# mako443/Text2Pos-CVPR2022

Hardware: AMD Instinct MI355X
Metric: cells+queries encoded/sec and top-k retrieval QPS, 256-pt cells, 12k-cell DB (higher is better)
Workload: dtype f16x3 (fp32 operands split hi+lo into fp16, 3 f16 MFMAs, fp32 accumulate; fp32-class error) for the encoders / f64 MFMA for the ranking

## Files before the change

include/t2p.h:

```cpp
#ifndef T2P_H
#define T2P_H
#include <stddef.h>
#include <stdint.h>

#ifdef __cplusplus
extern "C" {
#endif

#define T2P_ABI_VERSION 31
#define T2P_DEFAULT_CHUNK_OBJECTS 65000
#define T2P_MAX_CHUNK_OBJECTS 65535
#define T2P_TUNING_MASK 0x5
#define T2P_E_ARG (-1)
#define T2P_E_WORKSPACE (-2)
#define T2P_E_UNSUPPORTED (-3)

typedef void* t2p_stream_t;

int t2p_abi_version(void);
const char* t2p_last_error(void);

typedef struct t2p_cell_weights {
    const float* sa_w1[3];
    const float* sa_b1[3];
    const float* sa_w2[3];
    const float* sa_b2[3];
    const float* ga_w1;
    const float* ga_b1;
    const float* ga_w2;
    const float* ga_b2;
    const float* lin1_w;
    const float* lin1_b;
    const float* lin2_w;
    const float* lin2_b;
    const float* pn_w;
    const float* pn_b;
    const float* col_w1;
    const float* col_b1;
    const float* col_w2;
    const float* col_b2;
    const float* pos_w1;
    const float* pos_b1;
    const float* pos_w2;
    const float* pos_b2;
    const float* merge_w;
    const float* merge_b;
    const float* g_wp;
    const float* g_bp;
    const float* g_wq;
    const float* g_w2;
    const float* g_b2;
    const float* lin_w1;
    const float* lin_b1;
    const float* lin_w2;
    const float* lin_b2;
    const void* sa_w2_x3[3];
    const void* ga_w2_x3;
    const float* sa_b2_x3[3];
    float sa_w2_scale[3];
    const void* lin1_x3;
    const void* lin2_x3;
    const void* merge_x3;
    const void* pn_x3;
    const void* g_wp_x3;
    const void* g_wq_x3;
// ... 204 lines not shown
```

text2pos-cvpr2022_amd/csrc/api.hip:

```cpp
#include <stdarg.h>
#include <stdlib.h>
#include <string.h>

#include <mutex>
#include <set>
#include <utility>

#include "../../include/t2p.h"
#include "t2p_common.h"

namespace t2p {

static thread_local char g_err[512] = "";

void set_error(const char* fmt, ...) {
    va_list ap;
    va_start(ap, fmt);
    vsnprintf(g_err, sizeof(g_err), fmt, ap);
    va_end(ap);
}

int num_cus() {
    static int cached = 0;
    if (cached == 0) {
// ... 294 lines not shown
            p.k_live = Geo::C[l - 1] + 4;
            p.W = W.sa_w1[l];
            p.W_x3 = cfg.precision == 1 ? W.sa_w1_x3[l] : nullptr;
            p.ldw = H;
            p.bias = W.sa_b1[l];
            p.out = ws.A[l];
            p.ldo = H;
            p.relu = 0;
            p.M = n * g.nd[l];
            p.amax_out = gslot(l == 1 ? G_A2 : G_A3);
            T2P_TRY(launch_ws(WS_DENSE_STORE, Geo::LD[l - 1] - (cfg.precision == 1 ? 16 : 0), H, p, st));
        }
        SaParams p{};
        p.A = ws.A[l];
        p.Bc = ws.B[l];
        p.wp = lds_btab[l] ? W.sa_w1[l] + (size_t)cf * Geo::H[l] : nullptr;
        p.W = W.sa_w2[l];
        p.W_x3 = cfg.precision == 1 ? W.sa_w2_x3[l] : nullptr;
        p.bias = cfg.precision == 1 ? W.sa_b2_x3[l] : W.sa_b2[l];
        p.out_scale = cfg.precision == 1 ? 1.0f / W.sa_w2_scale[l] : 1.0f;
        p.out = ws.F[l];
        p.ldo = Geo::LD[l];
        p.rows = ws.gt.rows[l];
        p.n_rows = ws.gt.n_rows[l];
        p.first = ws.first;
        p.fps_idx = ws.gt.fps_idx[l];
        p.pos_src = pos_src;
        p.ld_pos = ld_pos;
        p.pos_col0 = pos_col0;
        if (l == 0 && sa1_points) {
            p.feat_src = rgb;
            p.w1 = W.sa_w1[0];
            p.b1 = W.sa_b1[0];
        }
        p.n_dense = g.nd[l];
        p.n_cent = g.nc[l];
        p.n_obj = n;
        p.prefix_ws = ws.prefix[l];
        p.bounds_ws = ws.bounds[l];
        p.balanced = 1;
        p.amax_out = gslot(G_F1 + l);
        if (l == 2) p.out_rows = g.gp;
        T2P_TRY(launch_ws_sa(H, C, p, st));
    }
    {
        WsParams p{};
        p.A = ws.F[2];
        p.lda = Geo::LD[2];
        p.W = W.ga_w1;
        p.W_x3 = cfg.precision == 1 ? W.ga_w1_x3 : nullptr;
        p.ldw = 512;
        p.bias = W.ga_b1;
        p.out = ws.gh;
        _Float16* gh_hi = (_Float16*)ws.gh;
        _Float16* gh_lo = gh_hi + (size_t)gh_rows(n, g) * 512;
        if (cfg.precision == 1) {
            p.out_hi = gh_hi;
            p.out_lo = gh_lo;
            p.amax_out = gslot(G_GA_H);
        }
        p.ldo = 512;
        p.relu = 1;
        p.M = n * g.gp;
        T2P_TRY(launch_ws(WS_DENSE_STORE, Geo::LD[2] - (cfg.precision == 1 ? 16 : 0), 512, p, st));
        WsParams q{};
        q.A = ws.gh;
        if (cfg.precision == 1) {
            q.A_hi = gh_hi;
            q.A_lo = gh_lo;
        }
        q.lda = 512;
        q.W = W.ga_w2;
        q.W_x3 = cfg.precision == 1 ? W.ga_w2_x3 : nullptr;
        q.ldw = 1024;
        q.bias = W.ga_b2;
        q.out = ws.f0;
        q.ldo = 1024;
        q.relu = 1;
        q.M = n * g.gp;
        q.group_rows = g.gp;
        T2P_TRY(launch_ws(WS_DENSE_GROUPMAX, 512, 1024, q, st));
    }
    if (cfg.precision == 1 && W.lin1_x3 && W.lin2_x3) {
        T2P_TRY(launch_gemm_x3(ws.f0, 1024, W.lin1_x3, W.lin1_scale, W.lin1_b, ws.f1, 512, 0, n, 1024, 512, 1, st, nullptr, 0, gslot(G_PN_F0)));
        T2P_TRY(launch_gemm_x3(ws.f1, 512, W.lin2_x3, W.lin2_scale, W.lin2_b, ws.f2, 256, 0, n, 512, 256, 1, st, nullptr, 0, gslot(G_PN_F1)));
    } else {
        T2P_TRY(launch_gemm(ws.f0, 1024, W.lin1_w, W.lin1_b, ws.f1, 512, 0, n, 1024, 512, 1, st));
        T2P_TRY(launch_gemm(ws.f1, 512, W.lin2_w, W.lin2_b, ws.f2, 256, 0, n, 512, 256, 1, st));
    }
    }
    if (trunk_only) {
        T2P_TRY(copy_trace(tr->features0, ws.f0, (size_t)n * 1024, st));
        T2P_TRY(copy_trace(tr->features1, ws.f1, (size_t)n * 512, st));
        T2P_TRY(copy_trace(tr->features2, ws.f2, (size_t)n * 256, st));
        T2P_TRY(launch_guard_check(guard, cfg.overflow_flag, gbounds, st));
        return 0;
    }
    const int nfeat = (cfg.use_class ? 1 : 0) + (cfg.use_color ? 1 : 0) + (cfg.use_position ? 1 : 0);
    const int ldcat = nfeat * D;
    int slot = 0;
    if (cfg.use_class && cfg.class_embed) {
        T2P_TRY(launch_gather_rownorm(W.class_embedding, cfg.class_idx + o_lo, n, D, ws.cat, ldcat, slot * D, st));
        slot++;
    } else if (cfg.use_class) {
        const float* fin = cfg.pointnet_features == 0 ? ws.f0 : (cfg.pointnet_features == 1 ? ws.f1 : ws.f2);
        const int kin = cfg.pointnet_features == 0 ? 1024 : (cfg.pointnet_features == 1 ? 512 : 256);
        if (cfg.precision == 1 && W.pn_x3)
            T2P_TRY(launch_gemm_x3(fin, kin, W.pn_x3, W.pn_scale, W.pn_b, ws.P, D, 0, n, kin, D, 1, st, nullptr, 0,
                                          gslot(G_PN_F0 + cfg.pointnet_features)));
        else
            T2P_TRY(launch_gemm(fin, kin, W.pn_w, W.pn_b, ws.P, D, 0, n, kin, D, 1, st));
        T2P_TRY(launch_rownorm(ws.P, D, n, D, ws.cat, ldcat, slot * D, st));
        slot++;
    }
    if (cfg.use_color && cfg.color_embed) {
        T2P_TRY(launch_gather_rownorm(W.color_embedding, cfg.color_idx + o_lo, n, D, ws.cat, ldcat, slot * D, st));
        slot++;
    } else if (cfg.use_color) {
        T2P_TRY(launch_mlp3_norm(mean_rgb, n, W.col_w1, W.col_b1, W.col_w2, W.col_b2, D, ws.cat, ldcat, slot * D, st));
        slot++;
    }
    if (cfg.use_position) {
// ... 665 lines not shown
```

text2pos-cvpr2022_amd/csrc/ga2.hip:

```cpp
#include "t2p_common.h"

namespace t2p {
namespace {


constexpr int K = 512, NW = 128, NT = 512;
constexpr int KH = K / 2;
constexpr int S16_FULL = K / 16;
constexpr int LDHH = K + 8;
constexpr int PLANE = 32 * LDHH;
constexpr int TILE_HALVES = 2 * PLANE;
constexpr int XCH_FLOATS = 4 * 16 * 64;
constexpr size_t kLds = (size_t)2 * TILE_HALVES * 2 + (size_t)XCH_FLOATS * 4;
constexpr int CHUNKS = (2 * 32 * (K / 8)) / NT;

template <int GP>
__global__ __launch_bounds__(NT, 2) void k_ga2(WsParams p, int n_slices) {
    extern __shared__ __attribute__((aligned(16))) float lds[];
    _Float16* tile = (_Float16*)lds;
    float* xch = (float*)(tile + 2 * TILE_HALVES);

    const int tid = threadIdx.x, lane = tid & 63, wave = tid >> 6;
    const int wn = wave & 3, kh = wave >> 2;

    const int lin = blockIdx.x, nblk = gridDim.x;
    int slice, stream, n_streams;
    if ((nblk % (8 * n_slices)) == 0) {
        const int xcd = lin & 7, j = lin >> 3, per_xcd = nblk >> 3;
        slice = j % n_slices;
        stream = xcd * (per_xcd / n_slices) + j / n_slices;
        n_streams = nblk / n_slices;
    } else {
        slice = lin % n_slices;
        stream = lin / n_slices;
        n_streams = nblk / n_slices;
    }
    const int ncol0 = slice * NW + wn * 32;

    constexpr int S32 = KH / 32;
    const int q16 = lane >> 4, i16 = lane & 15;
    half8 w_hi[2][S32], w_lo[2][S32];
    {
        const uint4* wp = (const uint4*)p.W_x3;
        const int plane_u4 = (p.ldw / 32) * S16_FULL * 64;
#pragma unroll
        for (int cb = 0; cb < 2; cb++)
#pragma unroll
            for (int s = 0; s < S32; s++) {
                const int idx = (((ncol0 / 32) * S16_FULL + (8 * q16 + s)) * 2 + kh) * 32 + 16 * cb + i16;
                w_hi[cb][s] = __builtin_bit_cast(half8, wp[idx]);
                w_lo[cb][s] = __builtin_bit_cast(half8, wp[plane_u4 + idx]);
            }
    }
    float bias2[2];
#pragma unroll
    for (int cb = 0; cb < 2; cb++) bias2[cb] = p.bias ? p.bias[ncol0 + 16 * cb + i16] : 0.f;

    typedef __attribute__((address_space(3))) void lds_void;
    typedef const __attribute__((address_space(1))) void gl_void;
    auto dma_piece = [&](int64_t g, int buf, int it) {
        const int q = it * (NT / 64) + wave;
        const int pl = q >> 5, row = q & 31;
        const _Float16* base = (const _Float16*)(pl ? p.A_lo : p.A_hi);
        const _Float16* src = base + (g * 32 + row) * (int64_t)p.lda + lane * 8;
        _Float16* dst = tile + buf * TILE_HALVES + pl * PLANE + row * LDHH;
        __builtin_amdgcn_global_load_lds((gl_void*)src, (lds_void*)dst, 16, 0, 0);
    };
    auto dma_tile = [&](int64_t g, int buf) {
#pragma unroll
        for (int it = 0; it < CHUNKS; it++) dma_piece(g, buf, it);
    };
    int64_t g = stream;
    if (g < p.n_groups) dma_tile(g, 0);
    __syncthreads();
    for (int i = 0; g < p.n_groups; g += n_streams, i++) {
        const int64_t gn = g + n_streams;
        const bool more = gn < p.n_groups;

        typedef float f32x4v __attribute__((ext_vector_type(4)));
        const f32x4v kZero4 = {0.f, 0.f, 0.f, 0.f};
        f32x4v acc[4], accx[4];
        const _Float16* hrow = tile + (i & 1) * TILE_HALVES + i16 * LDHH + kh * KH + q16 * 64;
        half8 a_hi[2], a_lo[2];
#pragma unroll
        for (int rb = 0; rb < 2; rb++) {
            a_hi[rb] = *(const half8*)(hrow + rb * 16 * LDHH);
            a_lo[rb] = *(const half8*)(hrow + PLANE + rb * 16 * LDHH);
        }
#pragma unroll
        for (int sl = 0; sl < 4 * S32; sl++) {
            const int s = sl >> 2, b = sl & 3, rb = b >> 1, cb = b & 1;
            __builtin_amdgcn_sched_barrier(0);
            if (s + 1 < S32 && b == 2) {
                a_hi[0] = *(const half8*)(hrow + (s + 1) * 8);
                a_lo[0] = *(const half8*)(hrow + PLANE + (s + 1) * 8);
            }
            if (s > 0 && b == 0) {
                a_hi[1] = *(const half8*)(hrow + 16 * LDHH + s * 8);
                a_lo[1] = *(const half8*)(hrow + PLANE + 16 * LDHH + s * 8);
            }
            acc[b] = __builtin_amdgcn_mfma_f32_16x16x32_f16(a_hi[rb], w_hi[cb][s], s == 0 ? kZero4 : acc[b], 0, 0, 0);
            accx[b] = __builtin_amdgcn_mfma_f32_16x16x32_f16(a_hi[rb], w_lo[cb][s], s == 0 ? kZero4 : accx[b], 0, 0, 0);
            accx[b] = __builtin_amdgcn_mfma_f32_16x16x32_f16(a_lo[rb], w_hi[cb][s], accx[b], 0, 0, 0);
            __builtin_amdgcn_sched_barrier(0);
            if (more && (sl & 1) == 0 && (sl >> 1) < CHUNKS) dma_piece(gn, (i + 1) & 1, sl >> 1);
        }
        __builtin_amdgcn_sched_barrier(0);
#pragma unroll
        for (int b = 0; b < 4; b++)
#pragma unroll
            for (int v = 0; v < 4; v++) acc[b][v] = fmaf(accx[b][v], 1.f / 2048.f, acc[b][v]);
        float* x = xch + wn * (16 * 64) + lane;
        const bool sender = ((i & 1) != 0) == (kh == 0);
        if (sender) {
#pragma unroll
            for (int b = 0; b < 4; b++)
#pragma unroll
                for (int v = 0; v < 4; v++) x[(4 * b + v) * 64] = acc[b][v];
        }
        __syncthreads();
        if (!sender && GP == 32) {
#pragma unroll
            for (int cb = 0; cb < 2; cb++) {
                float m = 0.f;
#pragma unroll
                for (int rb = 0; rb < 2; rb++)
#pragma unroll
                    for (int v = 0; v < 4; v++) m = fmaxf(m, (acc[2 * rb + cb][v] + x[(4 * (2 * rb + cb) + v) * 64]) + bias2[cb]);
                m = fmaxf(m, __shfl_xor(m, 16, 64));
                m = fmaxf(m, __shfl_xor(m, 32, 64));
                if (q16 == 0) p.out[g * (int64_t)p.ldo + ncol0 + 16 * cb + i16] = m;
            }
        } else if (!sender) {
            constexpr int VG = GP < 4 ? GP : 4;
            const int64_t n_obj = p.M / GP;
#pragma unroll
            for (int cb = 0; cb < 2; cb++)
#pragma unroll
                for (int rb = 0; rb < 2; rb++)
#pragma unroll
                    for (int v0 = 0; v0 < 4; v0 += VG) {
                        float m = 0.f;
#pragma unroll
                        for (int v = v0; v < v0 + VG; v++)
                            m = fmaxf(m, (acc[2 * rb + cb][v] + x[(4 * (2 * rb + cb) + v) * 64]) + bias2[cb]);
                        if constexpr (GP >= 8) m = fmaxf(m, __shfl_xor(m, 16, 64));
                        if constexpr (GP >= 16) m = fmaxf(m, __shfl_xor(m, 32, 64));
                        const int row = 16 * rb + 4 * q16 + v0;
                        const int64_t obj = g * (32 / GP) + row / GP;
                        if (row % GP == 0 && obj < n_obj) p.out[obj * (int64_t)p.ldo + ncol0 + 16 * cb + i16] = m;
                    }
        }
    }
}

template <int GP>
int launch_ga2_gp(const WsParams& p_in, hipStream_t st) {
    T2P_TRY(reserve_lds((const void*)k_ga2<GP>, kLds, "ga2"));
    WsParams p = p_in;
    p.n_groups = (p.M + 31) / 32;
    if (p.n_groups <= 0) return 0;
    const int n_slices = 1024 / NW;
    int64_t streams = matrix_wgs() / n_slices;
    if (streams < 1) streams = 1;
    if (streams > p.n_groups) streams = p.n_groups;
    if (streams >= 8) streams -= streams % 8;
    ProfScope ps_("ws_groupmax_k512_n1024", st);
    T2P_REPEAT(ps_) hipLaunchKernelGGL(k_ga2<GP>, dim3((unsigned)(streams * n_slices)), dim3(NT), kLds, st, p, n_slices);
    T2P_CHECK_LAUNCH("ga2");
    return 0;
}

}

int launch_ga2(const WsParams& p, hipStream_t st) {
    switch (p.group_rows > 0 ? p.group_rows : 32) {
        case 32: return launch_ga2_gp<32>(p, st);
        case 16: return launch_ga2_gp<16>(p, st);
        case 8: return launch_ga2_gp<8>(p, st);
        case 4: return launch_ga2_gp<4>(p, st);
        case 2: return launch_ga2_gp<2>(p, st);
        case 1: return launch_ga2_gp<1>(p, st);
    }
    set_error("ga2: group_rows=%d (1, 2, 4, 8, 16 or 32)", p.group_rows);
    return T2P_E_UNSUPPORTED;
}

}
```

text2pos-cvpr2022_amd/csrc/t2p_common.h:

```cpp
#pragma once
#include <hip/hip_runtime.h>
#include <stdint.h>
#include <stdio.h>

namespace t2p {

void set_error(const char* fmt, ...);

#define T2P_E_ARG (-1)
#define T2P_E_WORKSPACE (-2)
#define T2P_E_UNSUPPORTED (-3)

#define T2P_CHECK_ARG(cond, ...)                  \
    do {                                          \
        if (!(cond)) {                            \
            ::t2p::set_error(__VA_ARGS__);        \
            return T2P_E_ARG;                     \
        }                                         \
    } while (0)

#define T2P_CHECK_LAUNCH(name)                                                   \
    do {                                                                         \
        hipError_t e__ = hipGetLastError();                                      \
        if (e__ != hipSuccess) {                                                 \
// ... 156 lines not shown
                      const float* scene_center, const float* scene_color, int64_t n_out, int n_pts, float* xyz, float* rgb,
                      float* center, float* mean_rgb, int32_t* idx_out, hipStream_t st);
int launch_pairwise_ranking(const float* scores, int batch, float margin, float* row_loss, float* d_scores, float* row_cnt,
                            hipStream_t st);
int launch_hardest_ranking(const float* scores, int batch, float margin, float* best, int32_t* where, float* d_scores,
                           hipStream_t st);
int launch_cell_index(const int32_t* cell_ptr, int n_cells, int32_t o_lo, int32_t* seg_ptr_local, int32_t* first,
                      hipStream_t st, uint32_t* guard_to_clear = nullptr);

int launch_gemm(const float* A, int lda, const float* W, const float* bias, float* C, int ldc, int c0, int64_t M,
                int K, int N, int relu, hipStream_t st, const float* resid = nullptr, int ldr = 0);
int launch_gemm_skinny(const float* A, int lda, const float* W, float* C, int ldc, int64_t M, int K, int N, hipStream_t st);
int launch_gemm_x3(const float* A, int lda, const void* Wx, float scale, const float* bias, float* C, int ldc, int c0,
                   int64_t M, int K, int N, int relu, hipStream_t st, const float* resid = nullptr, int ldr = 0,
                   uint32_t* amax_in = nullptr );

size_t gemm_tn_workspace_bytes(int64_t M, int K1, int N);
int launch_edge_counts(const uint16_t* rows, const uint16_t* n_rows, const int32_t* first_obj, int64_t n_obj, int n_dense, int n_cent,
                       int self_loops, int32_t* counts, hipStream_t st);
int launch_edge_expand(const uint16_t* rows, const uint16_t* n_rows, const int32_t* first_obj, const int32_t* cent_ptr, int64_t n_obj,
                       int n_dense, int n_cent, int self_loops, int32_t* src, int32_t* dst, hipStream_t st);
size_t linear_wgrad_workspace_bytes(int64_t M, int K1, int N);
int launch_linear_wgrad_f32(const float* dY, int lda, const float* X, int ldb, float* dW, int ldc, float* colsum, int64_t M, int K1, int N,
                            void* ws, size_t ws_bytes, hipStream_t st);
int launch_gemm_tn(const float* A, int lda, const float* B, int ldb, float* C, int ldc, int64_t M, int K1, int N, void* ws,
                   size_t ws_bytes, hipStream_t st);

enum WsMode { WS_DENSE_STORE = 0, WS_DENSE_GROUPMAX = 1, WS_EDGE_KNN = 3 };
struct WsParams {
    const float* A;
    int lda;
    int k_live;
    const float* Bc;
    const float* W;
    int ldw;
    const void* W_x3;
    const void* A_hi;
    const void* A_lo;
    void* out_hi;
    void* out_lo;
    const float* bias;
    float* out;
    int ldo;
    int relu;
    int64_t n_groups;
    int64_t M;
    uint32_t* amax_out;
    const int32_t* knn_idx;
    int knn_k;
    int64_t n_dst;
    int mean;
    int knn_group;
    int group_rows;
};
int launch_ws(int mode, int K, int N, const WsParams& p, hipStream_t st);

struct SaParams {
    const float* A;
    const float* Bc;
    const float* wp;
    const float* W;
    const void* W_x3;
    const float* bias;
    float out_scale;
    float* out;
    int ldo;
    const uint16_t* rows;
    const uint16_t* n_rows;
    const int32_t* first;
    const uint8_t* fps_idx;
    const float* pos_src;
    int ld_pos, pos_col0;
    const float* feat_src;
    const float* w1;
    const float* b1;
    int n_dense, n_cent;
    int64_t n_obj;
    int32_t* prefix_ws;
    int32_t* bounds_ws;
    int balanced;
    uint32_t* amax_out;
    int out_rows;
};
int launch_ws_sa(int H, int C, const SaParams& p, hipStream_t st);
int launch_sa_balance(const SaParams& p, int tile_rows, int n_wg, hipStream_t st);
constexpr int kSaTailCode = 64;
bool sa_rows_selected(int H, int C, const SaParams& p);
int launch_sa_rows(int H, int C, const SaParams& p, hipStream_t st);
int sa_rows_launch_shape(int64_t n_obj, int* tile_rows, int* n_wg);
bool sa_points_selected(int H, int C, const SaParams& p);
int launch_sa_points(int H, int C, const SaParams& p, hipStream_t st);
int sa_points_launch_shape(int64_t n_obj, int* tile_rows, int* n_wg);
bool sa3_selected(int H, int C, const SaParams& p);
int launch_sa3(const SaParams& p, hipStream_t st);
int sa3_launch_shape(int64_t n_obj, int* tile_rows, int* n_wg);
inline bool sa_shares_tail_rows(int l, int H, int C, const SaParams& p, int n_pts, int tuning) {
    return l == 1 && n_pts == 256 && !(tuning & 4) && p.n_dense == 128 && p.n_cent == 64 && sa_rows_selected(H, C, p);
}
int launch_sa_balance_levels(const SaParams p[3], const int H[3], const int C[3], hipStream_t st);

int launch_bilstm_impl(const float* gate_table , const float* whh ,
                       const void* whh_x3 ,
                       float whh_scale, const int32_t* tokens , const int32_t* lengths, int B, int T, int V, int D,
                       float* hdir_ws , float* out ,
                       hipStream_t st);

int launch_lstm_cell_fwd(const float* pre, const float* table, const int32_t* tokens, const int32_t* lengths, int64_t B, int T,
// ... 37 lines not shown
```

text2pos-cvpr2022_amd/csrc/ws_gemm.hip:

```cpp
#ifndef T2P_GABL
#define T2P_GABL 0
#endif
#include <type_traits>

#include "t2p_common.h"

namespace t2p {
namespace {

constexpr int kMaxRows = 32 * 33;
constexpr int kAccFloats = 8192;

template <int K, int NW, int WN, int RT, int MODE, int X3, int W8 = 0>
struct WsCfg {
    static constexpr int NWAVES = (WN > 4 || W8) ? 8 : 4;
    static constexpr int NTH = 64 * NWAVES;
    static constexpr int WM = NWAVES / WN;
    static constexpr int NTW = NW / (32 * WN);
    static constexpr int KS = K / 2;
    static constexpr int TR = WM * RT * 32;
    static constexpr int LDH = K + 4;
    static constexpr int LDHH = K + 8;
    static constexpr int PLANE = TR * LDHH;
    static constexpr int S16 = K / 16;
    static constexpr bool EDGE = (MODE == WS_EDGE_KNN);
    static constexpr int TILE_FLOATS = X3 ? PLANE : TR * LDH;
    static constexpr int ACC_FLOATS = EDGE ? kAccFloats : 0;
    static constexpr int F4_PER_ROW = K / 4;
    static constexpr int TOTAL_F4 = TR * F4_PER_ROW;
    static constexpr int ITERS = (TOTAL_F4 + NTH - 1) / NTH;
    static constexpr size_t lds_bytes() {
        size_t b = (size_t)(2 * TILE_FLOATS + ACC_FLOATS) * 4;
        if (EDGE) b += (size_t)kMaxRows * 4 + kMaxRows + 40 * 4;
        return b;
    }
    static_assert(K % 8 == 0, "K must be a multiple of 8");
    static_assert(!X3 || K % 16 == 0, "f16x3 needs K % 16 == 0 (one MFMA step = 8 k per lane half)");
    static_assert(NW % (32 * WN) == 0, "NW must split into 32-column tiles per wave");
};

template <int K, int NW, int WN, int RT, int MODE, int X3, int SPLIT_IO, int W8 = 0, int GP = 32>
__global__ __launch_bounds__((WN > 4 || W8) ? 512 : 256, (WN > 4 || W8) ? 2 : 1) void k_ws(WsParams p, int n_slices) {
    using C = WsCfg<K, NW, WN, RT, MODE, X3, W8>;
    extern __shared__ __attribute__((aligned(16))) float lds[];
    float* hid = lds;
    _Float16* hidh = (_Float16*)lds;
    int* acc_lds = (int*)(lds + 2 * C::TILE_FLOATS);
    int* rows_src = (int*)(lds + 2 * C::TILE_FLOATS + C::ACC_FLOATS);
    uint8_t* rows_dst = (uint8_t*)(rows_src + kMaxRows);
    int* scan = (int*)(rows_dst + kMaxRows);

    const int tid = threadIdx.x, lane = tid & 63, wave = tid >> 6;
    const int wn = wave % WN, wm = wave / WN, h = lane >> 5, l31 = lane & 31;

    const int lin = blockIdx.x, nblk = gridDim.x;
    int slice, stream, n_streams;
    if ((nblk % (8 * n_slices)) == 0) {
        const int xcd = lin & 7, j = lin >> 3, per_xcd = nblk >> 3;
        slice = j % n_slices;
        stream = xcd * (per_xcd / n_slices) + j / n_slices;
        n_streams = nblk / n_slices;
    } else {
        slice = lin % n_slices;
        stream = lin / n_slices;
        n_streams = nblk / n_slices;
    }
    const int ncol0 = slice * NW + wn * C::NTW * 32;

    float w[X3 ? 1 : C::NTW][X3 ? 1 : C::KS];
    half8 w_hi[X3 ? C::NTW : 1][X3 ? C::S16 : 1], w_lo[X3 ? C::NTW : 1][X3 ? C::S16 : 1];
    if constexpr (X3) {
        const uint4* wp = (const uint4*)p.W_x3;
        const int plane_u4 = (p.ldw / 32) * C::S16 * 64;
#pragma unroll
        for (int nt = 0; nt < C::NTW; nt++)
#pragma unroll
            for (int s = 0; s < C::S16; s++) {
                const int idx = (((ncol0 / 32 + nt) * C::S16 + s) * 2 + h) * 32 + l31;
                const uint4 a = wp[idx], b = wp[plane_u4 + idx];
                w_hi[nt][s] = __builtin_bit_cast(half8, a);
                w_lo[nt][s] = __builtin_bit_cast(half8, b);
            }
    } else {
#pragma unroll
        for (int nt = 0; nt < C::NTW; nt++)
#pragma unroll
            for (int s = 0; s < C::KS; s++)
                w[nt][s] = p.W[(int64_t)(h * C::KS + s) * p.ldw + ncol0 + nt * 32 + l31];
    }
    float bias[C::NTW];
#pragma unroll
    for (int nt = 0; nt < C::NTW; nt++) bias[nt] = p.bias ? p.bias[ncol0 + nt * 32 + l31] : 0.f;

    const int k_live = p.k_live > 0 ? p.k_live : K;
    f32x4 sa[C::ITERS];
    f32x4 sb[C::EDGE ? C::ITERS : 1];

    const int knn_group = (C::EDGE && p.knn_group > 0) ? p.knn_group : 32;
    auto stage_load = [&](int64_t g, int r0, int n_rows) {
#pragma unroll
        for (int it = 0; it < C::ITERS; it++) {
            const int q = it * C::NTH + tid;
            const int lr = q / C::F4_PER_ROW, c4 = q % C::F4_PER_ROW;
            const int r = r0 + lr;
            sa[it] = f32x4{0.f, 0.f, 0.f, 0.f};
            if constexpr (C::EDGE) sb[it] = f32x4{0.f, 0.f, 0.f, 0.f};
            if (((C::TOTAL_F4 % C::NTH) == 0 || q < C::TOTAL_F4) && r < n_rows) {
                if constexpr (C::EDGE) {
                    const int src = rows_src[r];
                    const int dl = rows_dst[r];
                    if (dl != 0xFF) {
                        sa[it] = *(const f32x4*)(p.A + (int64_t)src * p.lda + c4 * 4);
                        sb[it] = *(const f32x4*)(p.Bc + (g * knn_group + dl) * K + c4 * 4);
                    }
                } else {
                    if (SPLIT_IO == 2 || c4 * 4 < k_live)
                        sa[it] = *(const f32x4*)(p.A + (g * C::TR + r) * (int64_t)p.lda + c4 * 4);
                }
            }
        }
    };
    float gmax_edge = 0.f;
    auto stage_write = [&](int buf) {
#pragma unroll
        for (int it = 0; it < C::ITERS; it++) {
            const int q = it * C::NTH + tid;
            if ((C::TOTAL_F4 % C::NTH) != 0 && q >= C::TOTAL_F4) break;
            const int lr = q / C::F4_PER_ROW, c4 = q % C::F4_PER_ROW;
            f32x4 v = sa[it];
            if constexpr (C::EDGE) {
                const f32x4 t = sa[it] + sb[it];
#pragma unroll
                for (int e = 0; e < 4; e++) v[e] = fmaxf(t[e], 0.f);
            }
            if constexpr (X3) {
                _Float16* dsth = hidh + buf * 2 * C::PLANE;
                if constexpr (C::EDGE)
                    gmax_edge = fmaxf(fmaxf(gmax_edge, fmaxf(v[0], v[1])), fmaxf(v[2], v[3]));
                const fp16x2 h01 = cvt_pk_f16(v[0], v[1]), h23 = cvt_pk_f16(v[2], v[3]);
                const fp16x2 l01 = cvt_pk_f16((v[0] - (float)h01[0]) * 2048.f, (v[1] - (float)h01[1]) * 2048.f);
                const fp16x2 l23 = cvt_pk_f16((v[2] - (float)h23[0]) * 2048.f, (v[3] - (float)h23[1]) * 2048.f);
                uint2 ph, pl;
                ph.x = __builtin_bit_cast(uint32_t, h01); ph.y = __builtin_bit_cast(uint32_t, h23);
                pl.x = __builtin_bit_cast(uint32_t, l01); pl.y = __builtin_bit_cast(uint32_t, l23);
                *(uint2*)(dsth + lr * C::LDHH + c4 * 4) = ph;
                *(uint2*)(dsth + C::PLANE + lr * C::LDHH + c4 * 4) = pl;
            } else {
                *(f32x4*)(hid + buf * C::TILE_FLOATS + lr * C::LDH + c4 * 4) = v;
            }
        }
    };
    auto mfma_block = [&](int buf, f32x16 (&acc)[RT][C::NTW]) {
#pragma unroll
        for (int rt = 0; rt < RT; rt++)
#pragma unroll
            for (int nt = 0; nt < C::NTW; nt++)
#pragma unroll
                for (int e = 0; e < 16; e++) acc[rt][nt][e] = bias[nt];
        if constexpr (X3) {
            f32x16 accx[RT][C::NTW];
#pragma unroll
            for (int rt = 0; rt < RT; rt++)
#pragma unroll
                for (int nt = 0; nt < C::NTW; nt++)
#pragma unroll
                    for (int e = 0; e < 16; e++) accx[rt][nt][e] = 0.f;
            const _Float16* hrow = hidh + buf * 2 * C::PLANE + ((wm * RT) * 32 + l31) * C::LDHH + h * (K / 2);
            half8 a_hi[RT], a_lo[RT], n_hi[RT], n_lo[RT];
#pragma unroll
            for (int rt = 0; rt < RT; rt++) {
                a_hi[rt] = *(const half8*)(hrow + rt * 32 * C::LDHH);
                a_lo[rt] = *(const half8*)(hrow + C::PLANE + rt * 32 * C::LDHH);
            }
#pragma unroll
            for (int s = 0; s < C::S16; s++) {
                if (s + 1 < C::S16) {
#pragma unroll
                    for (int rt = 0; rt < RT; rt++) {
                        n_hi[rt] = *(const half8*)(hrow + rt * 32 * C::LDHH + (s + 1) * 8);
                        n_lo[rt] = *(const half8*)(hrow + C::PLANE + rt * 32 * C::LDHH + (s + 1) * 8);
                    }
                }
                __builtin_amdgcn_sched_barrier(0);
#pragma unroll
                for (int rt = 0; rt < RT; rt++)
#pragma unroll
                    for (int nt = 0; nt < C::NTW; nt++) {
                        acc[rt][nt] = __builtin_amdgcn_mfma_f32_32x32x16_f16(a_hi[rt], w_hi[nt][s], acc[rt][nt], 0, 0, 0);
                        accx[rt][nt] = __builtin_amdgcn_mfma_f32_32x32x16_f16(a_hi[rt], w_lo[nt][s], accx[rt][nt], 0, 0, 0);
                    }
#pragma unroll
                for (int rt = 0; rt < RT; rt++)
#pragma unroll
                    for (int nt = 0; nt < C::NTW; nt++)
                        accx[rt][nt] = __builtin_amdgcn_mfma_f32_32x32x16_f16(a_lo[rt], w_hi[nt][s], accx[rt][nt], 0, 0, 0);
                __builtin_amdgcn_sched_barrier(0);
#pragma unroll
                for (int rt = 0; rt < RT; rt++) {
                    a_hi[rt] = n_hi[rt];
                    a_lo[rt] = n_lo[rt];
                }
            }
#pragma unroll
            for (int rt = 0; rt < RT; rt++)
#pragma unroll
                for (int nt = 0; nt < C::NTW; nt++)
#pragma unroll
                    for (int e = 0; e < 16; e++) acc[rt][nt][e] = fmaf(accx[rt][nt][e], 1.f / 2048.f, acc[rt][nt][e]);
        } else {
            const float* hrow = hid + buf * C::TILE_FLOATS + ((wm * RT) * 32 + l31) * C::LDH + h * C::KS;
            constexpr int NQ = C::KS / 4;
#pragma unroll
            for (int s4 = 0; s4 < NQ; s4++) {
                f32x4 a[RT];
#pragma unroll
                for (int rt = 0; rt < RT; rt++) a[rt] = *(const f32x4*)(hrow + rt * 32 * C::LDH + s4 * 4);
#pragma unroll
                for (int j = 0; j < 4; j++)
#pragma unroll
                    for (int rt = 0; rt < RT; rt++)
#pragma unroll
                        for (int nt = 0; nt < C::NTW; nt++)
                            acc[rt][nt] = __builtin_amdgcn_mfma_f32_32x32x2f32(a[rt][j], w[nt][s4 * 4 + j], acc[rt][nt],
                                                                                0, 0, 0);
            }
        }
    };

    if constexpr (!C::EDGE) {
        int64_t g = stream;
        auto rows_of = [&](int64_t gg) -> int {
            const int64_t left = p.M - gg * C::TR;
            return (int)(left < C::TR ? left : C::TR);
        };
        if (g < p.n_groups) {
            stage_load(g, 0, rows_of(g));
            stage_write(0);
        }
        __syncthreads();
        float gmax_all = 0.f;
        (void)gmax_all;
        for (int i = 0; g < p.n_groups; g += n_streams, i++) {
            const int64_t gn = g + n_streams;
            const int n_rows = rows_of(g);
            if (gn < p.n_groups) stage_load(gn, 0, rows_of(gn));
            f32x16 acc[RT][C::NTW];
            mfma_block(i & 1, acc);
            float gmax_out = 0.f;
            (void)gmax_out;
            auto epilogue = [&](auto full_tag) {
            constexpr bool FULL = decltype(full_tag)::value;
#pragma unroll
            for (int rt = 0; rt < RT; rt++) {
                const int trow0 = (wm * RT + rt) * 32;
#pragma unroll
                for (int nt = 0; nt < C::NTW; nt++) {
                    const int lcol = wn * C::NTW * 32 + nt * 32 + l31;
                    if constexpr (MODE == WS_DENSE_STORE) {
                        const int64_t o0 = (g * C::TR + trow0 + 4 * h) * (int64_t)p.ldo + slice * NW + lcol;
#pragma unroll
                        for (int e = 0; e < 16; e++) {
                            const int rr = (e & 3) + 8 * (e >> 2);
                            const int r = trow0 + 4 * h + rr;
                            float v = acc[rt][nt][e];
                            if (p.relu) v = fmaxf(v, 0.f);
                            if constexpr (X3) gmax_out = fmaxf(gmax_out, fabsf(v));
                            if constexpr (SPLIT_IO == 2) {
                                const fp16x2 hv = cvt_pk_f16(v, 0.f);
                                const fp16x2 lv = cvt_pk_f16((v - (float)hv[0]) * 2048.f, 0.f);
#if T2P_GABL & 1
                                if (FULL || r < n_rows) {
                                    ((__fp16*)p.out_hi + (o0 & 0xFFFFF))[rr * p.ldo] = hv[0];
                                    ((__fp16*)p.out_lo + (o0 & 0xFFFFF))[rr * p.ldo] = lv[0];
                                }
#else
                                if (FULL || r < n_rows) {
                                    ((__fp16*)p.out_hi + o0)[rr * p.ldo] = hv[0];
                                    ((__fp16*)p.out_lo + o0)[rr * p.ldo] = lv[0];
                                }
#endif
                            } else {
                                if (FULL || r < n_rows) (p.out + o0)[rr * p.ldo] = v;
                            }
                        }
                    } else if constexpr (GP == 32) {
                        float m = 0.f;
#pragma unroll
                        for (int e = 0; e < 16; e++) m = fmaxf(m, acc[rt][nt][e]);
                        m = fmaxf(m, __shfl_xor(m, 32, 64));
                        if (h == 0 && (FULL || trow0 < n_rows))
                            p.out[(g * (C::TR / 32) + wm * RT + rt) * (int64_t)p.ldo + slice * NW + lcol] = m;
                    } else {
                        constexpr int NG = 32 / GP;
                        float mg[NG];
#pragma unroll
                        for (int k = 0; k < NG; k++) mg[k] = 0.f;
#pragma unroll
                        for (int e = 0; e < 16; e++) {
                            const int k = (8 * (e >> 2) + (GP >= 8 ? 0 : (e & 3))) / GP;
                            mg[k] = fmaxf(mg[k], acc[rt][nt][e]);
                        }
                        const int64_t obj0 = (g * C::TR + trow0) / GP, n_obj = p.M / GP;
#pragma unroll
                        for (int k = 0; k < NG; k++) {
                            if constexpr (GP >= 8) {
                                const float m = fmaxf(mg[k], __shfl_xor(mg[k], 32, 64));
                                if (h == 0 && obj0 + k < n_obj) p.out[(obj0 + k) * (int64_t)p.ldo + slice * NW + lcol] = m;
                            } else if ((k * GP) % 8 < 4) {
                                const int64_t obj = obj0 + k + (4 / GP) * h;
                                if (obj < n_obj) p.out[obj * (int64_t)p.ldo + slice * NW + lcol] = mg[k];
                            }
                        }
                    }
                }
            }
            };
            if (n_rows == C::TR) epilogue(std::true_type{});
            else epilogue(std::false_type{});
            if constexpr (X3 && MODE == WS_DENSE_STORE) gmax_all = fmaxf(gmax_all, gmax_out);
            if (gn < p.n_groups) stage_write((i + 1) & 1);
            __syncthreads();
        }
        if constexpr (X3 && MODE == WS_DENSE_STORE) guard_publish_exact(p.amax_out, gmax_all);
    } else {
        for (int64_t g = stream; g < p.n_groups; g += n_streams) {
            const int64_t d0 = g * knn_group;
            const int nd = (int)((p.n_dst - d0) < knn_group ? (p.n_dst - d0) : knn_group);
            int my = 0;
            if (tid < nd)
                for (int e = 0; e < p.knn_k; e++) my += p.knn_idx[(d0 + tid) * p.knn_k + e] >= 0 ? 1 : 0;
            if (tid <= 32) scan[tid] = 0;
            __syncthreads();
            if (tid < 32) scan[tid + 1] = my;
// ... 47 lines not shown
                                const float other = __shfl_xor(sum, 32, 64);
                                sum = h == 0 ? sum + other : other + sum;
                                if (h == 0 && d < nd) {
                                    const int cnt = scan[d + 1] - scan[d];
                                    acc_lds[d * NW + lcol] = __float_as_int(cnt > 0 ? sum / (float)cnt : 0.f);
                                }
                            }
                        }
                        continue;
                    }
                    int dd[16];
                    bool same[16], is_end[16];
#pragma unroll
                    for (int e = 0; e < 16; e++) {
                        const int r = trow0 + 8 * (e >> 2) + 4 * h + (e & 3);
                        dd[e] = r < n_rows ? (int)rows_dst[r] : -1;
                    }
#pragma unroll
                    for (int e = 0; e < 16; e++) {
                        same[e] = e > 0 && dd[e] == dd[e - 1];
                        is_end[e] = dd[e] >= 0 && (e == 15 || dd[e] != dd[e + 1]);
                    }
#pragma unroll
                    for (int nt = 0; nt < C::NTW; nt++) {
                        const int lcol = wn * C::NTW * 32 + nt * 32 + l31;
                        float v[16];
#pragma unroll
                        for (int e = 0; e < 16; e++) {
                            v[e] = acc[rt][nt][e];
                            if (e > 0) v[e] = same[e] ? fmaxf(v[e], v[e - 1]) : v[e];
                        }
#pragma unroll
                        for (int e = 0; e < 16; e++)
                            if (is_end[e]) atomicMax(&acc_lds[dd[e] * NW + lcol], __float_as_int(v[e]));
                    }
                }
                if (more) stage_write((bt + 1) & 1);
                __syncthreads();
            }
            for (int i = tid; i < nd * NW; i += C::NTH) {
                const int c = i / NW, col = i % NW;
                p.out[(d0 + c) * (int64_t)p.ldo + slice * NW + col] = __int_as_float(acc_lds[i]);
            }
            __syncthreads();
        }
        if constexpr (X3) guard_publish_exact(p.amax_out, gmax_edge);
    }
}

template <int K, int NW, int WN, int RT, int MODE, int X3, int SPLIT_IO, int W8 = 0, int GP = 32>
int launch_cfg(const WsParams& p_in, int n_slices, hipStream_t st) {
    using C = WsCfg<K, NW, WN, RT, MODE, X3, W8>;
    auto kern = k_ws<K, NW, WN, RT, MODE, X3, SPLIT_IO, W8, GP>;
    T2P_TRY(reserve_lds((const void*)kern, C::lds_bytes(), "ws_gemm"));
    WsParams p = p_in;
    if (MODE != WS_EDGE_KNN) p.n_groups = (p.M + C::TR - 1) / C::TR;
    if (p.n_groups <= 0) return 0;
    const int cus = num_cus();
    int64_t streams = cus / n_slices;
    if (streams < 1) streams = 1;
    if (streams > p.n_groups) streams = p.n_groups;
    if (streams >= 8) streams -= streams % 8;
    const unsigned grid = (unsigned)(streams * n_slices);
    static const char* kMode[] = {"dense", "groupmax", "edge_sa", "edge_knn"};
    static char name[64];
    if (name[0] == 0) snprintf(name, sizeof(name), "ws_%s_k%d_n%d", kMode[MODE], K, NW * n_slices);
    ProfScope ps_(name, st);
    T2P_REPEAT(ps_) hipLaunchKernelGGL(kern, dim3(grid), dim3(C::NTH), C::lds_bytes(), st, p, n_slices);
    T2P_CHECK_LAUNCH("ws_gemm");
    return 0;
}

}

int launch_ga2(const WsParams& p, hipStream_t st);

int launch_ws(int mode, int K, int N, const WsParams& p, hipStream_t st) {
    T2P_CHECK_ARG((((uintptr_t)p.A | (uintptr_t)p.A_hi | (uintptr_t)p.A_lo) & 15) == 0 && (p.lda % 4) == 0,
                  "ws_gemm: A must be 16-byte aligned, lda %% 4 == 0");
    const int x3 = p.W_x3 != nullptr ? 1 : 0;
    if (x3) T2P_CHECK_ARG(((uintptr_t)p.W_x3 & 15) == 0, "ws_gemm: packed f16x3 weights must be 16-byte aligned");
    const int gp = p.group_rows > 0 ? p.group_rows : 32;
    if (mode == WS_DENSE_GROUPMAX)
        T2P_CHECK_ARG(gp <= 32 && (gp & (gp - 1)) == 0 && p.M % gp == 0, "ws_gemm: groupmax needs group_rows in {1, 2, 4, 8, 16, 32} "
                      "and M %% group_rows == 0 (group_rows=%d M=%lld)", p.group_rows, (long long)p.M);
    const int split_io = p.A_hi != nullptr ? 1 : (p.out_hi != nullptr ? 2 : 0);
    T2P_CHECK_ARG(split_io == 0 || x3 == 1, "ws_gemm: split fp16 activations need the f16x3 path");
    T2P_CHECK_ARG(p.k_live == 0 || (split_io == 0 && mode == WS_DENSE_STORE && p.k_live % 4 == 0),
                  "ws_gemm: k_live is honoured by the fp32-in / fp32-out dense mode only (multiple of 4)");
    if (split_io == 1) T2P_CHECK_ARG(p.A_lo != nullptr && p.lda % 8 == 0, "ws_gemm: split input needs both planes, lda %% 8 == 0");
    if (split_io == 2) T2P_CHECK_ARG(p.out_lo != nullptr, "ws_gemm: split output needs both planes");
#define WS_CASE(MODE_, K_, N_, NW_, WN_, RT_, X3_, SIO_)                                      \
    if (mode == MODE_ && K == K_ && N == N_ && x3 == X3_ && split_io == SIO_)                  \
        return launch_cfg<K_, NW_, WN_, RT_, MODE_, X3_, SIO_>(p, N_ / NW_, st);
    WS_CASE(WS_EDGE_KNN, 256, 256, 256, 8, 1, 0, 0)
    WS_CASE(WS_EDGE_KNN, 256, 256, 256, 8, 1, 1, 0)
    WS_CASE(WS_EDGE_KNN, 128, 128, 128, 4, 1, 0, 0)
    WS_CASE(WS_EDGE_KNN, 128, 128, 128, 4, 1, 1, 0)
    WS_CASE(WS_EDGE_KNN, 384, 384, 128, 4, 1, 0, 0)
    WS_CASE(WS_EDGE_KNN, 384, 384, 128, 4, 1, 1, 0)
    WS_CASE(WS_DENSE_STORE, 96, 128, 128, 4, 2, 0, 0)
    WS_CASE(WS_DENSE_STORE, 160, 256, 256, 4, 1, 0, 0)
    WS_CASE(WS_DENSE_STORE, 288, 512, 128, 4, 1, 0, 0)
    if (mode == WS_DENSE_STORE && K == 80 && N == 128 && x3 == 1 && split_io == 0)
        return launch_cfg<80, 128, 4, 1, WS_DENSE_STORE, 1, 0, 1>(p, 1, st);
    WS_CASE(WS_DENSE_STORE, 144, 256, 256, 8, 1, 1, 0)
    WS_CASE(WS_DENSE_STORE, 272, 512, 256, 8, 1, 1, 2)
    if (mode == WS_DENSE_GROUPMAX && K == 512 && N == 1024 && x3 == 0 && split_io == 0) {
        switch (gp) {
            case 32: return launch_cfg<512, 128, 4, 1, WS_DENSE_GROUPMAX, 0, 0>(p, 8, st);
            case 16: return launch_cfg<512, 128, 4, 1, WS_DENSE_GROUPMAX, 0, 0, 0, 16>(p, 8, st);
            case 8: return launch_cfg<512, 128, 4, 1, WS_DENSE_GROUPMAX, 0, 0, 0, 8>(p, 8, st);
            case 4: return launch_cfg<512, 128, 4, 1, WS_DENSE_GROUPMAX, 0, 0, 0, 4>(p, 8, st);
            case 2: return launch_cfg<512, 128, 4, 1, WS_DENSE_GROUPMAX, 0, 0, 0, 2>(p, 8, st);
            case 1: return launch_cfg<512, 128, 4, 1, WS_DENSE_GROUPMAX, 0, 0, 0, 1>(p, 8, st);
        }
    }
    if (mode == WS_DENSE_GROUPMAX && K == 512 && N == 1024 && x3 == 1 && split_io == 1) return launch_ga2(p, st);
    T2P_CHECK_ARG(mode != WS_DENSE_GROUPMAX || gp == 32, "ws_gemm: group_rows=%d is built for the fp32 and the ga2.hip paths", gp);
#undef WS_CASE
    set_error("ws_gemm: no instantiation for mode=%d K=%d N=%d x3=%d split_io=%d", mode, K, N, x3, split_io);
    return T2P_E_UNSUPPORTED;
}

}
```

Before: 155,100.

## Store GA hidden activations in chunk-ordered split fp16 layout for coalesced writes and reads

Adds a chunk-ordered layout for the split hi/lo fp16 hidden activations that sit between the two global-aggregation GEMMs. The producer GEMM swaps its MFMA operand order and uses permlane32 swaps so each lane writes 16-byte vectors rather than scattered 2-byte stores. The consumer ga2 kernel reads the planes without row padding. The layout is on by default (new tuning bit 8 disables it) and is meant to remove the strided scalar stores in the first GEMM's epilogue. In exchange it adds an LDS bias staging step and a new layout contract between the kernels, and the unpadded LDS reads could hit bank conflicts.

```diff
diff --git a/include/t2p.h b/include/t2p.h
--- a/include/t2p.h
+++ b/include/t2p.h
@@ -10,7 +10,7 @@
 #define T2P_ABI_VERSION 31
 #define T2P_DEFAULT_CHUNK_OBJECTS 65000
 #define T2P_MAX_CHUNK_OBJECTS 65535
-#define T2P_TUNING_MASK 0x5
+#define T2P_TUNING_MASK 0xD
 #define T2P_E_ARG (-1)
 #define T2P_E_WORKSPACE (-2)
 #define T2P_E_UNSUPPORTED (-3)
diff --git a/text2pos-cvpr2022_amd/csrc/api.hip b/text2pos-cvpr2022_amd/csrc/api.hip
--- a/text2pos-cvpr2022_amd/csrc/api.hip
+++ b/text2pos-cvpr2022_amd/csrc/api.hip
@@ -370,11 +370,13 @@
         p.ldw = 512;
         p.bias = W.ga_b1;
         p.out = ws.gh;
+        const int gh_chunks = (cfg.precision == 1 && !(cfg.tuning & 8)) ? 1 : 0;
         _Float16* gh_hi = (_Float16*)ws.gh;
         _Float16* gh_lo = gh_hi + (size_t)gh_rows(n, g) * 512;
         if (cfg.precision == 1) {
             p.out_hi = gh_hi;
             p.out_lo = gh_lo;
+            p.gh_chunks = gh_chunks;
             p.amax_out = gslot(G_GA_H);
         }
         p.ldo = 512;
@@ -386,6 +388,7 @@
         if (cfg.precision == 1) {
             q.A_hi = gh_hi;
             q.A_lo = gh_lo;
+            q.gh_chunks = gh_chunks;
         }
         q.lda = 512;
         q.W = W.ga_w2;
diff --git a/text2pos-cvpr2022_amd/csrc/ga2.hip b/text2pos-cvpr2022_amd/csrc/ga2.hip
--- a/text2pos-cvpr2022_amd/csrc/ga2.hip
+++ b/text2pos-cvpr2022_amd/csrc/ga2.hip
@@ -13,9 +13,13 @@
 constexpr int XCH_FLOATS = 4 * 16 * 64;
 constexpr size_t kLds = (size_t)2 * TILE_HALVES * 2 + (size_t)XCH_FLOATS * 4;
 constexpr int CHUNKS = (2 * 32 * (K / 8)) / NT;
+constexpr int PLANE_CH = 32 * K;
+static_assert(2 * 2 * PLANE_CH <= 2 * TILE_HALVES, "the chunk-ordered tiles fit the row-major tiles' LDS");
 
-template <int GP>
+template <int GP, int CH>
 __global__ __launch_bounds__(NT, 2) void k_ga2(WsParams p, int n_slices) {
+    constexpr int PL = CH ? PLANE_CH : PLANE;
+    constexpr int RB = CH ? 16 * 8 : 16 * LDHH;
     extern __shared__ __attribute__((aligned(16))) float lds[];
     _Float16* tile = (_Float16*)lds;
     float* xch = (float*)(tile + 2 * TILE_HALVES);
@@ -62,8 +66,8 @@
         const int q = it * (NT / 64) + wave;
         const int pl = q >> 5, row = q & 31;
         const _Float16* base = (const _Float16*)(pl ? p.A_lo : p.A_hi);
-        const _Float16* src = base + (g * 32 + row) * (int64_t)p.lda + lane * 8;
-        _Float16* dst = tile + buf * TILE_HALVES + pl * PLANE + row * LDHH;
+        const _Float16* src = CH ? base + g * (int64_t)(32 * K) + row * 512 + lane * 8 : base + (g * 32 + row) * (int64_t)p.lda + lane * 8;
+        _Float16* dst = tile + buf * TILE_HALVES + pl * PL + row * (CH ? 512 : LDHH);
         __builtin_amdgcn_global_load_lds((gl_void*)src, (lds_void*)dst, 16, 0, 0);
     };
     auto dma_tile = [&](int64_t g, int buf) {
@@ -80,24 +84,25 @@
         typedef float f32x4v __attribute__((ext_vector_type(4)));
         const f32x4v kZero4 = {0.f, 0.f, 0.f, 0.f};
         f32x4v acc[4], accx[4];
-        const _Float16* hrow = tile + (i & 1) * TILE_HALVES + i16 * LDHH + kh * KH + q16 * 64;
+        const _Float16* hrow = tile + (i & 1) * TILE_HALVES + (CH ? gh_chunk_index(0, 32 * kh + 8 * q16) * 8 + i16 * 8 : i16 * LDHH + kh * KH + q16 * 64);
+        auto ks = [](int s) { return CH ? gh_chunk_index(0, s) * 8 : s * 8; };
         half8 a_hi[2], a_lo[2];
 #pragma unroll
         for (int rb = 0; rb < 2; rb++) {
-            a_hi[rb] = *(const half8*)(hrow + rb * 16 * LDHH);
-            a_lo[rb] = *(const half8*)(hrow + PLANE + rb * 16 * LDHH);
+            a_hi[rb] = *(const half8*)(hrow + rb * RB);
+            a_lo[rb] = *(const half8*)(hrow + PL + rb * RB);
         }
 #pragma unroll
         for (int sl = 0; sl < 4 * S32; sl++) {
             const int s = sl >> 2, b = sl & 3, rb = b >> 1, cb = b & 1;
             __builtin_amdgcn_sched_barrier(0);
             if (s + 1 < S32 && b == 2) {
-                a_hi[0] = *(const half8*)(hrow + (s + 1) * 8);
-                a_lo[0] = *(const half8*)(hrow + PLANE + (s + 1) * 8);
+                a_hi[0] = *(const half8*)(hrow + ks(s + 1));
+                a_lo[0] = *(const half8*)(hrow + PL + ks(s + 1));
             }
             if (s > 0 && b == 0) {
-                a_hi[1] = *(const half8*)(hrow + 16 * LDHH + s * 8);
-                a_lo[1] = *(const half8*)(hrow + PLANE + 16 * LDHH + s * 8);
+                a_hi[1] = *(const half8*)(hrow + RB + ks(s));
+                a_lo[1] = *(const half8*)(hrow + PL + RB + ks(s));
             }
             acc[b] = __builtin_amdgcn_mfma_f32_16x16x32_f16(a_hi[rb], w_hi[cb][s], s == 0 ? kZero4 : acc[b], 0, 0, 0);
             accx[b] = __builtin_amdgcn_mfma_f32_16x16x32_f16(a_hi[rb], w_lo[cb][s], s == 0 ? kZero4 : accx[b], 0, 0, 0);
@@ -154,9 +159,12 @@
     }
 }
 
-template <int GP>
+template <int GP, int CH>
 int launch_ga2_gp(const WsParams& p_in, hipStream_t st) {
-    T2P_TRY(reserve_lds((const void*)k_ga2<GP>, kLds, "ga2"));
+    T2P_TRY(reserve_lds((const void*)k_ga2<GP, CH>, kLds, "ga2"));
+    if (CH)
+        T2P_CHECK_ARG(p_in.lda == K && (((uintptr_t)p_in.A_hi | (uintptr_t)p_in.A_lo) & 15) == 0,
+                      "ga2: chunk-ordered planes need lda == %d and 16-byte alignment", K);
     WsParams p = p_in;
     p.n_groups = (p.M + 31) / 32;
     if (p.n_groups <= 0) return 0;
@@ -166,7 +174,7 @@
     if (streams > p.n_groups) streams = p.n_groups;
     if (streams >= 8) streams -= streams % 8;
     ProfScope ps_("ws_groupmax_k512_n1024", st);
-    T2P_REPEAT(ps_) hipLaunchKernelGGL(k_ga2<GP>, dim3((unsigned)(streams * n_slices)), dim3(NT), kLds, st, p, n_slices);
+    T2P_REPEAT(ps_) hipLaunchKernelGGL((k_ga2<GP, CH>), dim3((unsigned)(streams * n_slices)), dim3(NT), kLds, st, p, n_slices);
     T2P_CHECK_LAUNCH("ga2");
     return 0;
 }
@@ -174,14 +182,11 @@
 }
 
 int launch_ga2(const WsParams& p, hipStream_t st) {
+#define GA2_CASE(GP_) case GP_: return p.gh_chunks ? launch_ga2_gp<GP_, 1>(p, st) : launch_ga2_gp<GP_, 0>(p, st);
     switch (p.group_rows > 0 ? p.group_rows : 32) {
-        case 32: return launch_ga2_gp<32>(p, st);
-        case 16: return launch_ga2_gp<16>(p, st);
-        case 8: return launch_ga2_gp<8>(p, st);
-        case 4: return launch_ga2_gp<4>(p, st);
-        case 2: return launch_ga2_gp<2>(p, st);
-        case 1: return launch_ga2_gp<1>(p, st);
+        GA2_CASE(32) GA2_CASE(16) GA2_CASE(8) GA2_CASE(4) GA2_CASE(2) GA2_CASE(1)
     }
+#undef GA2_CASE
     set_error("ga2: group_rows=%d (1, 2, 4, 8, 16 or 32)", p.group_rows);
     return T2P_E_UNSUPPORTED;
 }
diff --git a/text2pos-cvpr2022_amd/csrc/t2p_common.h b/text2pos-cvpr2022_amd/csrc/t2p_common.h
--- a/text2pos-cvpr2022_amd/csrc/t2p_common.h
+++ b/text2pos-cvpr2022_amd/csrc/t2p_common.h
@@ -232,7 +232,20 @@
     int mean;
     int knn_group;
     int group_rows;
-};
+    int gh_chunks;
+};
+__host__ __device__ constexpr int gh_chunk_index(int r, int c) { return (c >> 1) * 64 + (c & 1) * 32 + r; }
+constexpr bool gh_chunk_index_is_bijection() {
+    bool seen[32 * 64] = {};
+    for (int r = 0; r < 32; r++)
+        for (int c = 0; c < 64; c++) {
+            const int i = gh_chunk_index(r, c);
+            if (i < 0 || i >= 32 * 64 || seen[i]) return false;
+            seen[i] = true;
+        }
+    return true;
+}
+static_assert(gh_chunk_index_is_bijection(), "gh_chunk_index must map the 32 x 64 chunks of a tile onto [0, 2048) one to one");
 int launch_ws(int mode, int K, int N, const WsParams& p, hipStream_t st);
 
 struct SaParams {
diff --git a/text2pos-cvpr2022_amd/csrc/ws_gemm.hip b/text2pos-cvpr2022_amd/csrc/ws_gemm.hip
--- a/text2pos-cvpr2022_amd/csrc/ws_gemm.hip
+++ b/text2pos-cvpr2022_amd/csrc/ws_gemm.hip
@@ -1,6 +1,3 @@
-#ifndef T2P_GABL
-#define T2P_GABL 0
-#endif
 #include <type_traits>
 
 #include "t2p_common.h"
@@ -91,6 +88,11 @@
     float bias[C::NTW];
 #pragma unroll
     for (int nt = 0; nt < C::NTW; nt++) bias[nt] = p.bias ? p.bias[ncol0 + nt * 32 + l31] : 0.f;
+    float* bias_lds = lds + 2 * C::TILE_FLOATS + C::ACC_FLOATS;
+    if constexpr (SPLIT_IO == 3) {
+        static_assert(RT == 1 && C::NTW == 1 && MODE == WS_DENSE_STORE && X3 == 1, "chunk-ordered split output: one 32 x 32 block per wave");
+        for (int c = tid; c < NW; c += C::NTH) bias_lds[c] = p.bias ? p.bias[slice * NW + c] : 0.f;
+    }
 
     const int k_live = p.k_live > 0 ? p.k_live : K;
     f32x4 sa[C::ITERS];
@@ -114,7 +116,7 @@
                         sb[it] = *(const f32x4*)(p.Bc + (g * knn_group + dl) * K + c4 * 4);
                     }
                 } else {
-                    if (SPLIT_IO == 2 || c4 * 4 < k_live)
+                    if (SPLIT_IO >= 2 || c4 * 4 < k_live)
                         sa[it] = *(const f32x4*)(p.A + (g * C::TR + r) * (int64_t)p.lda + c4 * 4);
                 }
             }
@@ -157,6 +159,14 @@
             for (int nt = 0; nt < C::NTW; nt++)
 #pragma unroll
                 for (int e = 0; e < 16; e++) acc[rt][nt][e] = bias[nt];
+        if constexpr (SPLIT_IO == 3) {
+#pragma unroll
+            for (int q = 0; q < 4; q++) {
+                const f32x4 b4 = *(const f32x4*)(bias_lds + wn * 32 + 8 * q + 4 * h);
+#pragma unroll
+                for (int v = 0; v < 4; v++) acc[0][0][4 * q + v] = b4[v];
+            }
+        }
         if constexpr (X3) {
             f32x16 accx[RT][C::NTW];
 #pragma unroll
@@ -186,14 +196,23 @@
                 for (int rt = 0; rt < RT; rt++)
 #pragma unroll
                     for (int nt = 0; nt < C::NTW; nt++) {
-                        acc[rt][nt] = __builtin_amdgcn_mfma_f32_32x32x16_f16(a_hi[rt], w_hi[nt][s], acc[rt][nt], 0, 0, 0);
-                        accx[rt][nt] = __builtin_amdgcn_mfma_f32_32x32x16_f16(a_hi[rt], w_lo[nt][s], accx[rt][nt], 0, 0, 0);
+                        if constexpr (SPLIT_IO == 3) {
+                            acc[rt][nt] = __builtin_amdgcn_mfma_f32_32x32x16_f16(w_hi[nt][s], a_hi[rt], acc[rt][nt], 0, 0, 0);
+                            accx[rt][nt] = __builtin_amdgcn_mfma_f32_32x32x16_f16(w_lo[nt][s], a_hi[rt], accx[rt][nt], 0, 0, 0);
+                        } else {
+                            acc[rt][nt] = __builtin_amdgcn_mfma_f32_32x32x16_f16(a_hi[rt], w_hi[nt][s], acc[rt][nt], 0, 0, 0);
+                            accx[rt][nt] = __builtin_amdgcn_mfma_f32_32x32x16_f16(a_hi[rt], w_lo[nt][s], accx[rt][nt], 0, 0, 0);
+                        }
                     }
 #pragma unroll
                 for (int rt = 0; rt < RT; rt++)
 #pragma unroll
-                    for (int nt = 0; nt < C::NTW; nt++)
-                        accx[rt][nt] = __builtin_amdgcn_mfma_f32_32x32x16_f16(a_lo[rt], w_hi[nt][s], accx[rt][nt], 0, 0, 0);
+                    for (int nt = 0; nt < C::NTW; nt++) {
+                        if constexpr (SPLIT_IO == 3)
+                            accx[rt][nt] = __builtin_amdgcn_mfma_f32_32x32x16_f16(w_hi[nt][s], a_lo[rt], accx[rt][nt], 0, 0, 0);
+                        else
+                            accx[rt][nt] = __builtin_amdgcn_mfma_f32_32x32x16_f16(a_lo[rt], w_hi[nt][s], accx[rt][nt], 0, 0, 0);
+                    }
                 __builtin_amdgcn_sched_barrier(0);
 #pragma unroll
                 for (int rt = 0; rt < RT; rt++) {
@@ -250,6 +269,41 @@
             (void)gmax_out;
             auto epilogue = [&](auto full_tag) {
             constexpr bool FULL = decltype(full_tag)::value;
+            if constexpr (SPLIT_IO == 3) {
+                const int piece0 = (slice * NW + wn * 32) / 16;
+                static_assert(gh_chunk_index(5, 7) == 3 * 64 + 32 + 5, "the epilogue's addresses restate gh_chunk_index");
+                const int64_t o0 = g * C::TR * (int64_t)p.ldo + (int64_t)(piece0 * 64 + lane) * 8;
+                const bool ok = FULL || l31 < n_rows;
+#pragma unroll
+                for (int qp = 0; qp < 2; qp++) {
+                    uint32_t hd[2][2], ld[2][2];
+#pragma unroll
+                    for (int qq = 0; qq < 2; qq++) {
+                        float v[4];
+#pragma unroll
+                        for (int e = 0; e < 4; e++) {
+                            v[e] = acc[0][0][4 * (2 * qp + qq) + e];
+                            if (p.relu) v[e] = fmaxf(v[e], 0.f);
+                            gmax_out = fmaxf(gmax_out, fabsf(v[e]));
+                        }
+                        const fp16x2 h01 = cvt_pk_f16(v[0], v[1]), h23 = cvt_pk_f16(v[2], v[3]);
+                        const fp16x2 l01 = cvt_pk_f16((v[0] - (float)h01[0]) * 2048.f, (v[1] - (float)h01[1]) * 2048.f);
+                        const fp16x2 l23 = cvt_pk_f16((v[2] - (float)h23[0]) * 2048.f, (v[3] - (float)h23[1]) * 2048.f);
+                        hd[qq][0] = __builtin_bit_cast(uint32_t, h01); hd[qq][1] = __builtin_bit_cast(uint32_t, h23);
+                        ld[qq][0] = __builtin_bit_cast(uint32_t, l01); ld[qq][1] = __builtin_bit_cast(uint32_t, l23);
+                    }
+                    typedef unsigned u32x2_ __attribute__((ext_vector_type(2)));
+                    const u32x2_ h0 = __builtin_amdgcn_permlane32_swap(hd[0][0], hd[1][0], false, false);
+                    const u32x2_ h1 = __builtin_amdgcn_permlane32_swap(hd[0][1], hd[1][1], false, false);
+                    const u32x2_ l0 = __builtin_amdgcn_permlane32_swap(ld[0][0], ld[1][0], false, false);
+                    const u32x2_ l1 = __builtin_amdgcn_permlane32_swap(ld[0][1], ld[1][1], false, false);
+                    if (ok) {
+                        *(uint4*)((__fp16*)p.out_hi + o0 + qp * 512) = make_uint4(h0[0], h1[0], h0[1], h1[1]);
+                        *(uint4*)((__fp16*)p.out_lo + o0 + qp * 512) = make_uint4(l0[0], l1[0], l0[1], l1[1]);
+                    }
+                }
+                return;
+            }
 #pragma unroll
             for (int rt = 0; rt < RT; rt++) {
                 const int trow0 = (wm * RT + rt) * 32;
@@ -268,17 +322,10 @@
                             if constexpr (SPLIT_IO == 2) {
                                 const fp16x2 hv = cvt_pk_f16(v, 0.f);
                                 const fp16x2 lv = cvt_pk_f16((v - (float)hv[0]) * 2048.f, 0.f);
-#if T2P_GABL & 1
-                                if (FULL || r < n_rows) {
-                                    ((__fp16*)p.out_hi + (o0 & 0xFFFFF))[rr * p.ldo] = hv[0];
-                                    ((__fp16*)p.out_lo + (o0 & 0xFFFFF))[rr * p.ldo] = lv[0];
-                                }
-#else
                                 if (FULL || r < n_rows) {
                                     ((__fp16*)p.out_hi + o0)[rr * p.ldo] = hv[0];
                                     ((__fp16*)p.out_lo + o0)[rr * p.ldo] = lv[0];
                                 }
-#endif
                             } else {
                                 if (FULL || r < n_rows) (p.out + o0)[rr * p.ldo] = v;
                             }
@@ -432,7 +479,8 @@
 int launch_cfg(const WsParams& p_in, int n_slices, hipStream_t st) {
     using C = WsCfg<K, NW, WN, RT, MODE, X3, W8>;
     auto kern = k_ws<K, NW, WN, RT, MODE, X3, SPLIT_IO, W8, GP>;
-    T2P_TRY(reserve_lds((const void*)kern, C::lds_bytes(), "ws_gemm"));
+    constexpr size_t kLdsBytes = C::lds_bytes() + (SPLIT_IO == 3 ? NW * 4 : 0);
+    T2P_TRY(reserve_lds((const void*)kern, kLdsBytes, "ws_gemm"));
     WsParams p = p_in;
     if (MODE != WS_EDGE_KNN) p.n_groups = (p.M + C::TR - 1) / C::TR;
     if (p.n_groups <= 0) return 0;
@@ -446,7 +494,7 @@
     static char name[64];
     if (name[0] == 0) snprintf(name, sizeof(name), "ws_%s_k%d_n%d", kMode[MODE], K, NW * n_slices);
     ProfScope ps_(name, st);
-    T2P_REPEAT(ps_) hipLaunchKernelGGL(kern, dim3(grid), dim3(C::NTH), C::lds_bytes(), st, p, n_slices);
+    T2P_REPEAT(ps_) hipLaunchKernelGGL(kern, dim3(grid), dim3(C::NTH), kLdsBytes, st, p, n_slices);
     T2P_CHECK_LAUNCH("ws_gemm");
     return 0;
 }
@@ -464,12 +512,15 @@
     if (mode == WS_DENSE_GROUPMAX)
         T2P_CHECK_ARG(gp <= 32 && (gp & (gp - 1)) == 0 && p.M % gp == 0, "ws_gemm: groupmax needs group_rows in {1, 2, 4, 8, 16, 32} "
                       "and M %% group_rows == 0 (group_rows=%d M=%lld)", p.group_rows, (long long)p.M);
-    const int split_io = p.A_hi != nullptr ? 1 : (p.out_hi != nullptr ? 2 : 0);
+    const int split_io = p.A_hi != nullptr ? 1 : (p.out_hi != nullptr ? (p.gh_chunks ? 3 : 2) : 0);
     T2P_CHECK_ARG(split_io == 0 || x3 == 1, "ws_gemm: split fp16 activations need the f16x3 path");
     T2P_CHECK_ARG(p.k_live == 0 || (split_io == 0 && mode == WS_DENSE_STORE && p.k_live % 4 == 0),
                   "ws_gemm: k_live is honoured by the fp32-in / fp32-out dense mode only (multiple of 4)");
     if (split_io == 1) T2P_CHECK_ARG(p.A_lo != nullptr && p.lda % 8 == 0, "ws_gemm: split input needs both planes, lda %% 8 == 0");
-    if (split_io == 2) T2P_CHECK_ARG(p.out_lo != nullptr, "ws_gemm: split output needs both planes");
+    if (split_io >= 2) T2P_CHECK_ARG(p.out_lo != nullptr, "ws_gemm: split output needs both planes");
+    if (split_io == 3)
+        T2P_CHECK_ARG((((uintptr_t)p.out_hi | (uintptr_t)p.out_lo) & 15) == 0 && p.ldo % 16 == 0 && p.ldo >= N,
+                      "ws_gemm: chunk-ordered planes must be 16-byte aligned, ldo %% 16 == 0");
 #define WS_CASE(MODE_, K_, N_, NW_, WN_, RT_, X3_, SIO_)                                      \
     if (mode == MODE_ && K == K_ && N == N_ && x3 == X3_ && split_io == SIO_)                  \
         return launch_cfg<K_, NW_, WN_, RT_, MODE_, X3_, SIO_>(p, N_ / NW_, st);
@@ -486,6 +537,7 @@
         return launch_cfg<80, 128, 4, 1, WS_DENSE_STORE, 1, 0, 1>(p, 1, st);
     WS_CASE(WS_DENSE_STORE, 144, 256, 256, 8, 1, 1, 0)
     WS_CASE(WS_DENSE_STORE, 272, 512, 256, 8, 1, 1, 2)
+    WS_CASE(WS_DENSE_STORE, 272, 512, 256, 8, 1, 1, 3)
     if (mode == WS_DENSE_GROUPMAX && K == 512 && N == 1024 && x3 == 0 && split_io == 0) {
         switch (gp) {
             case 32: return launch_cfg<512, 128, 4, 1, WS_DENSE_GROUPMAX, 0, 0>(p, 8, st);
```

Result: no change. 156,300 (median of 6 runs) (+0.8%).
